# robertknight/ocrs

Hardware: AMD Instinct MI355X
Metric: pages/sec end-to-end (1024x1024) (higher is better)
Workload: dtype f32

## Files before the change

### include/ocrs_amd.h

```cpp
#ifndef OCRS_AMD_H
#define OCRS_AMD_H

#include <stddef.h>
#include <stdint.h>

#if defined(__GNUC__)
#define OCRS_API __attribute__((visibility("default")))
#else
#define OCRS_API
#endif

#ifdef __cplusplus
extern "C" {
#endif

typedef enum ocrs_status {
    OCRS_OK = 0,
    OCRS_ERR_INVALID_ARGUMENT = 1,
    OCRS_ERR_MODEL_NOT_LOADED = 2,
    OCRS_ERR_MODEL_DIMS = 3,
    OCRS_ERR_RUN_FAILED = 4,
    OCRS_ERR_WRONG_OUTPUT = 5,
    OCRS_ERR_IMAGE_SOURCE = 6,
    OCRS_ERR_DEVICE = 7,
    OCRS_ERR_IO = 8,
    OCRS_ERR_CAPACITY = 9
} ocrs_status;

OCRS_API const char* ocrs_last_error(void);

#define OCRS_ABI_VERSION 6u
OCRS_API uint32_t ocrs_abi_version(void);

OCRS_API void ocrs_buffer_free(void* p);

OCRS_API ocrs_status ocrs_device_count(int* n);
OCRS_API ocrs_status ocrs_set_device(int device);
OCRS_API ocrs_status ocrs_get_device(int* device);

OCRS_API ocrs_status ocrs_ctc_beam_search(const float* logp, int t, int c, uint32_t width, int impl, uint32_t** labels,
                                          uint32_t** positions, size_t* n);
OCRS_API ocrs_status ocrs_ctc_beam_search_scored(const float* logp, int t, int c, uint32_t width, int impl, uint32_t** labels,
                                                 uint32_t** positions, size_t* n, double* score, float** step_logp);

OCRS_API ocrs_status ocrs_gru_tile_plan(const int32_t* lengths_desc, size_t n_lines, int hidden, int32_t* n_clusters, int32_t* waves,
                                        int16_t* tiles);

OCRS_API ocrs_status ocrs_coalescer_selftest(int n_threads, int requests_per_thread, int max_active, int max_pages,
                                             long window_us, int fail_every, uint64_t out[5]);

OCRS_API ocrs_status ocrs_set_option(const char* name, long value);
OCRS_API ocrs_status ocrs_option_name(int index, const char** name);

OCRS_API ocrs_status ocrs_device_pool_stats(int device, uint64_t out[12]);
OCRS_API ocrs_status ocrs_device_pool_configure(int device, uint64_t device_cached_cap_bytes, uint64_t pinned_cached_cap_bytes);
OCRS_API ocrs_status ocrs_device_pool_trim(int device);

typedef enum { OCRS_ISOLATION_AUTO = 0, OCRS_ISOLATION_NONE = 1 } ocrs_isolation;
OCRS_API ocrs_status ocrs_device_set_isolation(int device, ocrs_isolation policy);
OCRS_API ocrs_status ocrs_device_isolation(int device, int out[3]);

typedef struct ocrs_model ocrs_model;

OCRS_API ocrs_status ocrs_model_load_file(const char* path, ocrs_model** out);
OCRS_API ocrs_status ocrs_model_load_bytes(const void* data, size_t len, ocrs_model** out);
OCRS_API ocrs_status ocrs_model_load_file_on_device(const char* path, int device, ocrs_model** out);
OCRS_API ocrs_status ocrs_model_load_bytes_on_device(const void* data, size_t len, int device, ocrs_model** out);
OCRS_API ocrs_status ocrs_model_device(const ocrs_model* m, int* device);

// ... 214 lines not shown
```

### ocrs_amd/_lib.py

```python
import ctypes as C
import os

_HERE = os.path.dirname(os.path.abspath(__file__))
LIB_PATH = os.environ.get("OCRS_AMD_LIB") or os.path.join(_HERE, "libocrs_amd.so")

OCRS_OK = 0
STATUS_NAMES = {
    0: "OK", 1: "INVALID_ARGUMENT", 2: "MODEL_NOT_LOADED", 3: "MODEL_DIMS", 4: "RUN_FAILED", 5: "WRONG_OUTPUT",
    6: "IMAGE_SOURCE", 7: "DEVICE", 8: "IO", 9: "CAPACITY",
}

RUN_FN = C.CFUNCTYPE(C.c_int, C.c_void_p, C.POINTER(C.c_float), C.POINTER(C.c_int64), C.POINTER(C.POINTER(C.c_float)),
                     C.POINTER(C.c_int64), C.POINTER(C.c_int))


class EngineParams(C.Structure):
    _fields_ = [("detection_model", C.c_void_p), ("recognition_model", C.c_void_p), ("debug", C.c_int),
                ("decode_method", C.c_int), ("beam_width", C.c_uint32), ("alphabet", C.c_char_p),
                ("allowed_chars", C.c_char_p), ("numerics", C.c_int), ("coalesce", C.c_int), ("coalesce_pages", C.c_int),
                ("coalesce_window_us", C.c_int), ("layout_threads", C.c_int), ("rec_max_pixels", C.c_int64)]


class GroupParams(C.Structure):
    _fields_ = [("detection_model", C.c_void_p), ("detection_model_len", C.c_size_t), ("recognition_model", C.c_void_p),
# ... 12 lines not shown
    _fields_ = [("ch", C.c_uint32), ("top", C.c_int32), ("left", C.c_int32), ("bottom", C.c_int32),
                ("right", C.c_int32)]


class OcrsError(RuntimeError):
    def __init__(self, status, message):
        super().__init__(message)
        self.status = status
        self.status_name = STATUS_NAMES.get(status, str(status))


DECLARED_SYMBOLS = [
    "ocrs_last_error", "ocrs_buffer_free", "ocrs_device_count", "ocrs_set_device", "ocrs_set_option", "ocrs_ctc_beam_search", "ocrs_model_load_file",
    "ocrs_model_load_bytes", "ocrs_model_from_callback", "ocrs_model_input_shape", "ocrs_model_run",
    "ocrs_model_flops", "ocrs_model_free", "ocrs_engine_new", "ocrs_engine_free", "ocrs_image_source_check_bytes",
    "ocrs_engine_prepare_input", "ocrs_engine_prepare_input_device", "ocrs_page_free", "ocrs_page_dims",
    "ocrs_page_image", "ocrs_engine_detect_words", "ocrs_engine_detect_words_batch",
    "ocrs_engine_detect_text_pixels", "ocrs_engine_detection_threshold", "ocrs_engine_find_text_lines",
    "ocrs_engine_find_text_lines_batch",
    "ocrs_engine_recognize_text", "ocrs_engine_recognize_text_batch", "ocrs_engine_recognize_tokens",
    "ocrs_engine_prepare_recognition_input", "ocrs_text_item_rotated_rect", "ocrs_rotated_rect_corners", "ocrs_engine_get_text", "ocrs_device_malloc", "ocrs_device_free",
    "ocrs_device_upload", "ocrs_device_synchronize", "ocrs_device_measure_peaks", "ocrs_engine_enable_timing", "ocrs_stage_count",
    "ocrs_stage_name", "ocrs_engine_stage_times", "ocrs_kernel_class_count", "ocrs_kernel_class_name",
    "ocrs_engine_kernel_stats", "ocrs_engine_set_kernel_timing_mask", "ocrs_gru_tile_plan", "ocrs_host_malloc", "ocrs_host_free", "ocrs_engine_prepare_input_batch",
    "ocrs_get_device", "ocrs_model_load_file_on_device", "ocrs_model_load_bytes_on_device", "ocrs_model_device", "ocrs_engine_device",
    "ocrs_engine_group_new", "ocrs_engine_group_free", "ocrs_engine_group_size", "ocrs_engine_group_member", "ocrs_group_deal",
    "ocrs_group_prepare_input_batch", "ocrs_group_prepare_input_device_batch", "ocrs_group_detect_words_batch",
    "ocrs_group_recognize_text_batch", "ocrs_group_gather", "ocrs_group_final_gather", "ocrs_group_worker_threads", "ocrs_group_last_gather", "ocrs_device_malloc_on", "ocrs_engine_coalesce_stats", "ocrs_coalescer_selftest", "ocrs_engine_kernel_mfma_flops", "ocrs_engine_prepare_input_jpeg", "ocrs_jpeg_decode_rgb", "ocrs_jpeg_info", "ocrs_jpeg_coefficients",
    "ocrs_group_member_stats", "ocrs_numa_parse_cpulist", "ocrs_numa_bind_selftest", "ocrs_engine_recognize_logits", "ocrs_engine_set_option", "ocrs_engine_get_option", "ocrs_option_name", "ocrs_device_pool_stats", "ocrs_device_pool_configure", "ocrs_device_pool_trim",
    "ocrs_device_set_isolation", "ocrs_device_isolation", "ocrs_group_set_replay", "ocrs_abi_version",
    "ocrs_engine_recognize_text_scored", "ocrs_engine_recognize_text_batch_scored", "ocrs_ctc_beam_search_scored",
    "ocrs_engine_run_recognition_ops",
]

ABI_VERSION = 6

_lib = None


def lib():
    global _lib
    if _lib is None:
        if not os.path.exists(LIB_PATH):
            raise OcrsError(7, "libocrs_amd.so is not built: run `python -m ocrs_amd.build` "
                               "(there is no CPU fallback for the HIP engine)")
        L = C.CDLL(LIB_PATH)
        L.ocrs_abi_version.restype = C.c_uint32
# ... 145 lines not shown
```

### ocrs_amd/csrc/abi.cpp

```cpp
#include <cstdio>
#include <fstream>
#include <thread>

#include <atomic>
#include "abi_util.hpp"
#include "coalesce_selftest.hpp"
#include "engine.hpp"
#include "host_pool.hpp"
#include "jpeg.hpp"
#include "kernels.hpp"

using namespace ocrs;
using namespace ocrs::geom;

using namespace ocrs::abi;

extern "C" {

const char* ocrs_last_error(void) { return last_error().c_str(); }

void ocrs_buffer_free(void* p) { free(p); }

ocrs_status ocrs_device_count(int* n) {
    return guarded([&] {
// ... 7 lines not shown
ocrs_status ocrs_set_device(int device) {
    return guarded([&] { select_device(device); });
}

ocrs_status ocrs_get_device(int* device) {
    return guarded([&] {
        if (!device) fail(OCRS_ERR_INVALID_ARGUMENT, "null argument");
        *device = default_device();
    });
}

ocrs_status ocrs_gru_tile_plan(const int32_t* lengths_desc, size_t n_lines, int hidden, int32_t* n_clusters, int32_t* waves,
                               int16_t* tiles) {
    return guarded([&] {
        if (!lengths_desc || !n_clusters || !waves || !tiles || n_lines == 0 || n_lines > (size_t)1 << 20)
            fail(OCRS_ERR_INVALID_ARGUMENT, "bad argument");
        for (size_t i = 0; i < n_lines; i++)
            if (lengths_desc[i] < 1 || (i > 0 && lengths_desc[i] > lengths_desc[i - 1]))
                fail(OCRS_ERR_INVALID_ARGUMENT, "lengths must be positive and descending");
        int ncl = 0;
        if (!k::gru_tile_plan(lengths_desc, (int)n_lines, hidden, &ncl, waves, tiles))
            fail(OCRS_ERR_CAPACITY, "no persistent-kernel plan for this shape (the engine then runs the recurrence as one fused launch per time step)");
        *n_clusters = ncl;
    });
}

ocrs_status ocrs_coalescer_selftest(int n_threads, int requests_per_thread, int max_active, int max_pages, long window_us,
                                    int fail_every, uint64_t out[5]) {
    return guarded([&] {
        if (!out || n_threads < 1 || requests_per_thread < 1 || max_pages < 1) fail(OCRS_ERR_INVALID_ARGUMENT, "bad argument");
        coalescer_selftest(n_threads, requests_per_thread, max_active, max_pages, window_us, fail_every, out);
    });
}

namespace {

void beam_search_hook(const float* logp, int t, int c, uint32_t width, int impl, std::vector<uint32_t>* l,
                      std::vector<uint32_t>* p, double* score, std::vector<float>* step_logp) {
    if (impl == 2 && t > 0) {
        DeviceScope bind(-1);
        if (!k::ctc_beam_supported(c, (int)width)) fail(OCRS_ERR_CAPACITY, "beam search on the GPU supports up to 128 classes and width 128");
        Workspace ws;
        std::vector<int32_t> meta(1 + t + 1);
        meta[0] = t;
        for (int i = 0; i <= t; i++) meta[1 + i] = i;
        int32_t* d_meta = ws.alloc_n<int32_t>(meta.size());
// ... 868 lines not shown
```

### ocrs_amd/csrc/common.cpp

```cpp
#include "common.hpp"

#include <chrono>
#include <climits>
#include <cstdint>
#include <cstdlib>
#include <cstring>

#include <algorithm>
#include <atomic>
#include <condition_variable>
#include <deque>
#include <system_error>

namespace ocrs {

static thread_local std::string g_last_error;

void set_last_error(const std::string& msg) { g_last_error = msg; }
const std::string& last_error() { return g_last_error; }

namespace {
std::atomic<int> g_default_device{0};
thread_local DeviceContext* t_ctx = nullptr;
constexpr int kMaxDevices = 64;
// ... 369 lines not shown
int DeviceContext::cu_count() {
    std::lock_guard<std::mutex> g(lazy_mu_);
    if (!cus_) {
        hipDeviceProp_t prop;
        OCRS_HIP(hipGetDeviceProperties(&prop, device));
        cus_ = prop.multiProcessorCount;
    }
    return cus_;
}

namespace {
struct OptDef { const char* name; const char* env; long def; };
const OptDef kOptDefs[OPT_COUNT] = {
    {"gru_mode", "OCRS_GRU_MODE", GRU_PERSISTENT},
    {"gru_gates", "OCRS_GRU_GATES", 1},
    {"gru_local", "OCRS_GRU_LOCAL", 1},
    {"det_fuse", "OCRS_DET_FUSE", 1},
    {"det_stream", "OCRS_DET_STREAM", 1},
    {"det_rows", "OCRS_DET_ROWS", 1},
    {"ccl_quad", "OCRS_CCL_QUAD", 1},
    {"conv12_fuse", "OCRS_CONV12_FUSE", 1},
    {"conv_flat", "OCRS_CONV_FLAT", 1},
    {"beam_gpu", "OCRS_BEAM_GPU", 1},
    {"numerics", nullptr, 0},
    {"coalesce", nullptr, 2},
    {"coalesce_pages", nullptr, 16},
    {"coalesce_window_us", nullptr, 300},
    {"layout_threads", nullptr, 0},
    {"rec_max_pixels", nullptr, 0},
};
struct OptRange { long lo, hi; long also[4]; };
const OptRange kOptRanges[OPT_COUNT] = {
    {0, 1, {}}, {0, 1, {}}, {0, 1, {}}, {0, 2, {}}, {0, 1, {8, 14, 32}}, {0, 1, {8, 14, 20, 32}}, {0, 1, {}}, {0, 1, {}}, {0, 1, {}}, {0, 1, {}},
    {0, 2, {}}, {0, 64, {}}, {1, 4096, {}}, {0, 10000000, {}}, {0, 4096, {}}, {0, INT64_MAX, {}},
};
bool in_range(int i, long v) {
    const OptRange& r = kOptRanges[i];
    if (v >= r.lo && v <= r.hi) return true;
    for (long a : r.also) if (a && v == a) return true;
    return false;
}
const char* const kRetired[] = {"det_heavy", "det_tail", "gru_waves", "gru_background", "gru_scatter", "gru_gates_pack", "conv_occupancy",
                                "gx_heavy", "gemm_nfast", "conv_a_lds", "gru_heavy", "heavy_priority", "det_mfma"};
std::atomic<long> g_opts[OPT_COUNT];
std::once_flag g_opts_once;
void init_options() {
    for (int i = 0; i < OPT_COUNT; i++) {
        const char* e = kOptDefs[i].env ? getenv(kOptDefs[i].env) : nullptr;
        const long v = e && *e ? strtol(e, nullptr, 10) : kOptDefs[i].def;
        g_opts[i].store(in_range(i, v) ? v : kOptDefs[i].def);
    }
}
int find_option(const char* name, int count = OPT_PUBLIC_COUNT) {
    for (int i = 0; i < count; i++)
        if (name && i != OPT_NUMERICS && strcmp(name, kOptDefs[i].name) == 0) return i;
    return -1;
// ... 173 lines not shown
```

### ocrs_amd/csrc/common.hpp

```cpp
#pragma once
#include <atomic>
#include <hip/hip_runtime.h>

#include <cstdarg>
#include <cstdint>
#include <cstdio>
#include <cstdlib>
#include <chrono>
#include <condition_variable>
#include <cstring>
#include <map>
#include <mutex>
#include <stdexcept>
#include <string>
#include <thread>
#include <vector>

#include "../../include/ocrs_amd.h"

namespace ocrs {

struct Error : std::runtime_error {
    ocrs_status status;
    Error(ocrs_status s, const std::string& msg) : std::runtime_error(msg), status(s) {}
// ... 94 lines not shown

DeviceContext& device_context(int device);
int default_device();
void select_device(int device);
DeviceContext& ctx();

class DeviceScope {
  public:
    explicit DeviceScope(int device);
    ~DeviceScope();
    DeviceScope(const DeviceScope&) = delete;
    DeviceScope& operator=(const DeviceScope&) = delete;

  private:
    DeviceContext* prev_;
    int restore_ = -1;
};

inline DevicePool& pool() { return ctx().pool; }
inline HostPool& host_pool() { return ctx().host_pool; }
inline hipStream_t heavy_stream() { return ctx().heavy_stream(); }

enum Option { OPT_GRU_MODE = 0, OPT_GRU_GATES, OPT_GRU_LOCAL, OPT_DET_FUSE, OPT_DET_STREAM, OPT_DET_ROWS, OPT_CCL_QUAD,
              OPT_CONV12_FUSE, OPT_CONV_FLAT, OPT_BEAM_GPU, OPT_PUBLIC_COUNT,
              OPT_NUMERICS = OPT_PUBLIC_COUNT,
              OPT_COALESCE, OPT_COALESCE_PAGES, OPT_COALESCE_WINDOW_US,
              OPT_LAYOUT_THREADS, OPT_REC_MAX_PIXELS,
              OPT_COUNT };
struct Tuning { long v[OPT_COUNT]; };
Tuning default_tuning();
int set_option(const char* name, long value);
int set_option(Tuning& t, const char* name, long value);
bool get_option(const Tuning& t, const char* name, long* value);
const char* option_name(int i);
class TuningScope {
  public:
    explicit TuningScope(const Tuning* t);
    ~TuningScope();
    TuningScope(const TuningScope&) = delete;
    TuningScope& operator=(const TuningScope&) = delete;
  private:
    const Tuning* prev_;
};
const Tuning* current_tuning();
enum { GRU_PERSISTENT = 0, GRU_STEP = 1 };
int option(Option o);

// ... 192 lines not shown
```

### ocrs_amd/csrc/kernels.hpp

```cpp
#pragma once
#include <vector>
#include <hip/hip_runtime.h>

#include <cstdint>

namespace ocrs {
namespace jpeg { struct Coefficients; }
namespace k {

void prepare_image(const void* d_pixels, bool is_u8, bool chans_last, int h, int w, int chans, float* d_out,
                   hipStream_t s);
void resize_pages_to_model(const float* const* d_src_ptrs, int n, int sh, int sw, int vh, int vw, float* d_dst,
                           int dh, int dw, hipStream_t s);
bool resize_threshold(const float* d_prob, int n, int mh, int mw, int sh, int sw, float thr, uint8_t* d_mask,
                      float* d_map, int h, int w, hipStream_t s, int32_t* d_labels = nullptr, int32_t* d_zero_a = nullptr,
                      int32_t* d_zero_b = nullptr);
void threshold_only(const float* d_prob, float thr, uint8_t* d_mask, int64_t count, hipStream_t s);

struct CclBuffers {
    int32_t* labels;
    int32_t* row_counts;
    int32_t* row_offsets;
    int32_t* n_roots;
    int32_t* roots;
// ... 67 lines not shown
void padcat(const float* skip, int n, int sh, int sw, int cs, const float* x, int h, int w, int cx, float* y,
            hipStream_t s);
void sigmoid(const float* x, float* y, int64_t count, hipStream_t s);
void conv1x1_cout1(const float* x, int64_t pixels, int cin, const float* wt, const float* bias, int relu, int do_sigmoid,
                   float* y, hipStream_t s);
void to_seq(const float* x, int n, int w, int c, float* y, hipStream_t s);
void gru_gates(const float* gx, const float* gh, float* h, float* y, int T, int N, int H, int step, hipStream_t s);
bool log_softmax_argmax(const float* logits, int64_t rows, int c, const uint8_t* d_excluded ,
                        float* logp, int32_t* labels, hipStream_t s, float* maxlp = nullptr);
void to_seq_packed(const float* x, int n, int T, int c, const int32_t* d_pos, const int32_t* d_off, float* y,
                   hipStream_t s);
void gru_gates_packed(const float* gx, const float* gh, float* h, float* y, const int32_t* d_Tm, const int32_t* d_off,
                      int64_t R, int Mcap, int active, int H, int step, hipStream_t s);
bool gru_step_fused(const float* gx, const float* wh, const float* bh, const float* hT_in, float* hT_out, float* y,
                    const int32_t* d_Tm, const int32_t* d_off, int64_t R, int Mcap, int active, int H, int step,
                    hipStream_t s);
size_t gru_persistent_sync_words(int M);
size_t gru_persistent_exchange_bytes(const int32_t* h_Tm, int M, int H);
bool gru_persistent_supported(const int32_t* h_Tm, int M, int Tmax, int64_t R, int H);
bool gru_tile_plan(const int32_t* h_Tm, int M, int H, int* ncl, int* waves, int16_t* tiles );
hipError_t gru_persistent_prepare(float* hx, const int32_t* h_Tm, int M, int H, hipStream_t s);
bool gru_persistent(const float* gx, const float* wh, const float* bh, float* y, float* hx, const int32_t* d_Tm, const int32_t* d_off,
                    const int32_t* h_Tm, int64_t R, int M, int Tmax, int H, uint32_t* d_sync, hipStream_t s);
bool gru_general_tile_plan(const int32_t* h_Tm, int M, int Tmax, int H, int cap, int* ncl, int16_t* tiles , int kernel );
size_t gru_split_exchange_bytes(const int32_t* h_Tm, int M, int H, int np);
bool gru_split_supported(const int32_t* h_Tm, int M, int Tmax, int64_t R, int H, int np);
hipError_t gru_split_prepare(uint16_t* hx, const int32_t* h_Tm, int M, int H, int np, hipStream_t s);
bool gru_persistent_split(const float* gx, const float* wh, const float* bh, float* y, uint16_t* hx, const int32_t* d_Tm, const int32_t* d_off,
                          const int32_t* h_Tm, int64_t R, int M, int Tmax, int H, int np, uint32_t* d_sync, hipStream_t s);
void ctc_collapse_packed(const int32_t* labels, const int32_t* d_Tm, const int32_t* d_off, int M, int Tmax,
                         uint32_t* out_labels, uint32_t* out_pos, int32_t* out_count, hipStream_t s);
void ctc_collapse_scored_packed(const int32_t* labels, const float* maxlp, const int32_t* d_Tm, const int32_t* d_off, int M,
                                int Tmax, uint32_t* out_labels, uint32_t* out_pos, float* out_logp, int32_t* out_count,
                                double* out_score, hipStream_t s);
void argmax_rows(const float* x, int64_t rows, int c, const uint8_t* d_excluded, int32_t* labels, hipStream_t s);
bool ctc_beam_supported(int C, int width);
size_t ctc_beam_arena_entries(int Tmax, int width);
bool ctc_beam_packed(const float* logp, const int32_t* d_Tm, const int32_t* d_off, int M, int Tmax, int C, int width,
                     const uint8_t* d_excluded, int2* d_nodes, int2* d_posn, uint32_t* out_labels, uint32_t* out_pos,
                     int32_t* out_count, hipStream_t s, double* out_score = nullptr, float* out_logp = nullptr);
void ctc_collapse(const int32_t* labels, int T, int N, uint32_t* out_labels, uint32_t* out_pos, int32_t* out_count,
                  hipStream_t s);

struct RaggedView {
    int G;
    int H;
// ... 57 lines not shown
```

### ocrs_amd/csrc/kernels_gru.hip

```cpp
#include <algorithm>
#include <cstdlib>
#include <map>
#include <mutex>
#include <vector>

#include "common.hpp"
#include "kernels.hpp"
#include "spec_math.hpp"

namespace ocrs {
namespace k {

typedef float f32x4 __attribute__((ext_vector_type(4)));
typedef unsigned u32x2 __attribute__((ext_vector_type(2)));

namespace {

constexpr int kMaxSlots = 128;

struct GruParams {
    const float* gx;
    const float* wh;
    const float* bh;
    float* y;
// ... 311 lines not shown
        if (!early) issue_state<H>(hxb, ub, kq, nxt);
        if (!await_state<H>(p, hxb, ub, kq, nxt)) return -1;
#ifdef OCRS_GRU_PROBE
        pr_wait += __builtin_readcyclecounter() - pt3;
#endif
        s = ns;
        i = ni;
        return 1;
    };
    for (;;) {
        if (item(bufA, bufB) <= 0) break;
        if (item(bufB, bufA) <= 0) break;
    }
#ifdef OCRS_GRU_PROBE
    if (cid == 0 && ub == 0 && lane == 0)
        printf("probe fp32 wave %d local %d tiles %d: items %llu, cycles per item %llu = transposes + issue %llu | chain %llu | gates + stores %llu | wait %llu\n", wave, (int)local,
               (t0 >= 0) + (t1 >= 0) + (t2 >= 0) + (t3 >= 0), (unsigned long long)pr_items, (unsigned long long)((__builtin_readcyclecounter() - pr_t0) / pr_items),
               (unsigned long long)(pr_tr / pr_items), (unsigned long long)(pr_mma / pr_items), (unsigned long long)(pr_gate / pr_items), (unsigned long long)(pr_wait / pr_items));
#endif
}



template <int H>
__device__ __forceinline__ f32x4 gate_chain(int lane, const float (&w)[H / 4], const float* lds_w, int g, const f32x4& bias) {
    f32x4 acc = bias;
    const f32x4* ap = reinterpret_cast<const f32x4*>(lds_w) + g * (H / 16) * 64 + lane;
    f32x4 a = ap[0];
#pragma unroll
    for (int blk = 0; blk < H / 16; blk++) {
        f32x4 na = a;
        if (blk + 1 < H / 16) na = ap[(blk + 1) * 64];
#pragma unroll
        for (int e = 0; e < 4; e++) acc = __builtin_amdgcn_mfma_f32_16x16x4f32(a[e], w[4 * blk + e], acc, 0, 0, 0);
        a = na;
    }
    return acc;
}

template <int H, bool FAST>
__global__ void __launch_bounds__(256)
gru_gates_kernel(GruParams p) {
    extern __shared__ __attribute__((aligned(16))) float lds_w[];
    asm volatile("v_accvgpr_write_b32 a200, 0" ::: "a200");
    constexpr int UB = H / 16;
    const int b = blockIdx.x;
// ... 108 lines not shown
                const float rg = sigmoid_g<FAST>(gr[r] + a.r[r]);
                const float zg = sigmoid_g<FAST>(gz[r] + a.z[r]);
                const float ng = tanh_g<FAST>(fmaf(rg, a.n[r], gn[r]));
                const float hv = fmaf(zg, hp[r] - ng, ng);
                hn[r] = __float_as_uint(hv) == kUnwritten ? __uint_as_float(0x7FC00000u) : hv;
            }
            const uint32_t o = active ? ((blk0 + s) * (H / 16) + ub) * 1024u + i16 * 64u + kq * 16u : 0xFFFFFFF0u;
            float t[4];
            transpose4(hn, t);
            const f32x4 ht = {t[0], t[1], t[2], t[3]};
            if (local) store_local(hxb, o, ht);
            else store_through(hxb, o, ht);
            store_local(yb, active ? out_off : 0xFFFFFFF0u, hn);
            if (active) hp = hn;
            gr = ngr; gz = ngz; gn = ngn; out_off = nout_off; active = nactive;
        }
    }
}


}

constexpr int kMaxGrid = 4096;
static size_t gru_gates_lds_bytes(int H, int Tmax) {
    return (size_t)H * 48 * sizeof(float) + (size_t)(((Tmax + 1) + 3) & ~3) * sizeof(int) + 3 * 64 * 16 + 16;
}
static size_t gru_general_lds_bytes(int H, int Tmax) { return (size_t)H * 48 * sizeof(float) + ((size_t)Tmax + 1) * sizeof(int); }
size_t gru_persistent_sync_words(int) { return kMaxGrid + 1; }

static int64_t gru_tile_blocks(const int32_t* h_Tm, int M) {
    int64_t tb = 0;
    for (int m = 0; m < M; m += 16) tb += h_Tm[m];
    return tb;
}
size_t gru_persistent_exchange_bytes(const int32_t* h_Tm, int M, int H) { return (size_t)2 * (size_t)gru_tile_blocks(h_Tm, M) * 16 * H * sizeof(float); }

hipError_t gru_persistent_prepare(float* hx, const int32_t* h_Tm, int M, int H, hipStream_t s) {
    return M > 0 ? hipMemsetAsync(hx, 0xFF, gru_persistent_exchange_bytes(h_Tm, M, H), s) : hipSuccess;
}

static int gru_resident_capacity(int H, bool gates, size_t lds) {
    static std::mutex mu;
    static std::map<int, int> cache;
    int dev = 0;
    if (hipGetDevice(&dev) != hipSuccess) return 0;
    const int key = dev * 8 + (gates ? 4 : 0) + (H == 256 ? 2 : H == 128 ? 1 : 0);
    {
        std::lock_guard<std::mutex> g(mu);
        auto it = cache.find(key);
        if (it != cache.end()) return it->second;
    }
    hipDeviceProp_t prop;
    if (hipGetDeviceProperties(&prop, dev) != hipSuccess) return 0;
    int per_cu = 0;
    hipError_t e;
    if (gates) {
        e = H == 256 ? hipOccupancyMaxActiveBlocksPerMultiprocessor(&per_cu, gru_gates_kernel<256, false>, 256, lds)
          : H == 128 ? hipOccupancyMaxActiveBlocksPerMultiprocessor(&per_cu, gru_gates_kernel<128, false>, 256, lds)
                     : hipOccupancyMaxActiveBlocksPerMultiprocessor(&per_cu, gru_gates_kernel<64, false>, 256, lds);
    } else {
        e = H == 256 ? hipOccupancyMaxActiveBlocksPerMultiprocessor(&per_cu, gru_persistent_kernel<256, false>, 256, lds)
          : H == 128 ? hipOccupancyMaxActiveBlocksPerMultiprocessor(&per_cu, gru_persistent_kernel<128, false>, 256, lds)
                     : hipOccupancyMaxActiveBlocksPerMultiprocessor(&per_cu, gru_persistent_kernel<64, false>, 256, lds);
    }
    if (e != hipSuccess) { (void)hipGetLastError(); per_cu = 0; }
    const int cap = prop.multiProcessorCount * (per_cu > 0 ? 1 : 0);
    std::lock_guard<std::mutex> g(mu);
    cache[key] = cap;
    return cap;
}

static bool gru_plan(int M, int Tmax, int H, int* ncl, int max_blocks = 256) {
    if (H != 256 && H != 128 && H != 64) return false;
    const int ntiles = (M + 15) / 16;
    const int UB = H / 16;
    max_blocks = max_blocks > 256 ? 256 : max_blocks;
    max_blocks -= max_blocks % (8 * UB);
    if (max_blocks < 8 * UB) return false;
    int max_ncl = max_blocks / UB / 2;
    if (ntiles > 16 * max_ncl) max_ncl *= 2;
    if (ntiles > 16 * max_ncl || 4 * max_ncl > kMaxSlots) return false;
    *ncl = (ntiles + 3) / 4 < max_ncl ? (ntiles + 3) / 4 : max_ncl;
    return gru_general_lds_bytes(H, Tmax) <= 64 * 1024;
}

static const int kRoundCost[3][5] = {{0, 63, 101, 150, 200}, {0, 54, 91, 128, 170}, {0, 44, 68, 99, 135}};
static void gru_assign_tiles(const int32_t* h_Tm, int M, int ncl, int16_t* tiles, int kernel = 0) {
    const int ntiles = (M + 15) / 16, nslots = 4 * ncl;
    const int* round = kRoundCost[kernel >= 0 && kernel < 3 ? kernel : 0];
    for (int i = 0; i < nslots * 4; i++) tiles[i] = -1;
    std::vector<int> cnt(nslots, 0);
    auto cost = [&](int slot, int extra_len) {
        int64_t tot = 0;
        int len[5], n = cnt[slot];
        for (int i = 0; i < n; i++) len[i] = h_Tm[tiles[slot * 4 + i] * 16];
        if (extra_len > 0) len[n++] = extra_len;
        for (int i = n - 1, below = 0; i >= 0; i--) {
            tot += (int64_t)(len[i] - below) * round[i + 1];
            below = len[i];
        }
        return tot;
    };
    for (int k = 0; k < ntiles; k++) {
        const int len = h_Tm[k * 16];
        int best = -1;
        int64_t best_cost = 0;
        for (int sl = 0; sl < nslots; sl++) {
            if (cnt[sl] >= 4) continue;
            const int64_t cs = cost(sl, len);
            if (best < 0 || cs < best_cost) { best = sl; best_cost = cs; }
        }
        tiles[best * 4 + cnt[best]++] = (int16_t)k;
    }
}

bool gru_tile_plan(const int32_t* h_Tm, int M, int H, int* ncl, int* waves, int16_t* tiles ) {
    for (int i = 0; i < kMaxSlots * 4; i++) tiles[i] = -1;
    *waves = 4;
    if (M <= 0 || !gru_plan(M, h_Tm[0], H, ncl, 256)) return false;
    gru_assign_tiles(h_Tm, M, *ncl, tiles);
    return true;
}

bool gru_general_tile_plan(const int32_t* h_Tm, int M, int Tmax, int H, int cap, int* ncl, int16_t* tiles, int kernel) {
    if (M <= 0 || !gru_plan(M, Tmax, H, ncl, cap)) return false;
    if (tiles) gru_assign_tiles(h_Tm, M, *ncl, tiles, kernel);
    return true;
}

bool gru_persistent_supported(const int32_t* h_Tm, int M, int Tmax, int64_t R, int H) {
    int ncl;
    if (H != 256 && H != 128 && H != 64) return false;
    return M > 0 && (uint64_t)R * 2 * H * sizeof(float) < (uint64_t(1) << 32) && (uint64_t)gru_persistent_exchange_bytes(h_Tm, M, H) < (uint64_t(1) << 32) &&
           gru_plan(M, Tmax, H, &ncl, gru_resident_capacity(H, false, gru_general_lds_bytes(H, Tmax)));
}

static bool gru_gates_plan(int M, int Tmax, int H, int* ncl) {
    if (H != 256 && H != 128 && H != 64) return false;
    if (gru_gates_lds_bytes(H, Tmax) > 64 * 1024) return false;
    const int ntiles = (M + 15) / 16, UB = H / 16;
    int cap = gru_resident_capacity(H, true, gru_gates_lds_bytes(H, Tmax));
    cap = cap > 256 ? 256 : cap;
    cap -= cap % (8 * UB);
    if (cap < 8 * UB || ntiles > cap / UB / 2) return false;
    *ncl = ntiles;
    return true;
}

template <int H>
static void launch_gates(bool fast, dim3 grid, size_t lds, hipStream_t s, const GruParams& g) {
    if (fast) hipLaunchKernelGGL((gru_gates_kernel<H, true>), grid, dim3(256), lds, s, g);
    else hipLaunchKernelGGL((gru_gates_kernel<H, false>), grid, dim3(256), lds, s, g);
}
template <int H>
static void launch_general(bool fast, dim3 grid, size_t lds, hipStream_t s, const GruParams& g) {
    if (fast) hipLaunchKernelGGL((gru_persistent_kernel<H, true>), grid, dim3(256), lds, s, g);
    else hipLaunchKernelGGL((gru_persistent_kernel<H, false>), grid, dim3(256), lds, s, g);
}

bool gru_persistent(const float* gx, const float* wh, const float* bh, float* y, float* hx, const int32_t* d_Tm, const int32_t* d_off,
                    const int32_t* h_Tm, int64_t R, int M, int Tmax, int H, uint32_t* d_sync, hipStream_t s) {
    if (M <= 0) return true;
    if (!hx || !gru_persistent_supported(h_Tm, M, Tmax, R, H)) return false;
    const bool fast = option(OPT_NUMERICS) != 0;
    GruParams p{};
    p.gx = gx; p.wh = wh; p.bh = bh; p.y = y; p.hx = hx; p.Tm = d_Tm; p.off = d_off;
    std::vector<int32_t> base((M + 15) / 16 + 1, 0);
    for (size_t k = 0; k + 1 < base.size(); k++) base[k + 1] = base[k] + h_Tm[k * 16];
    p.TB = base.back();
    p.place = d_sync;
    p.sync = d_sync + kMaxGrid;
    p.R = R; p.M = M; p.Tmax = Tmax;
    p.prio = 3;
    p.spin_limit = 1u << 21;
    p.allow_local = option(OPT_GRU_LOCAL) != 0;
    const int UB = H / 16;
    if (option(OPT_GRU_GATES) && gru_gates_plan(M, Tmax, H, &p.ncl)) {
        for (int k = 0; k < p.ncl; k++) p.tbase[k] = base[k];
        const dim3 grid(8 * UB * ((2 * p.ncl + 7) / 8));
        const size_t lds = gru_gates_lds_bytes(H, Tmax);
        OCRS_HIP(hipMemsetAsync(d_sync, 0, gru_persistent_sync_words(M) * sizeof(uint32_t), s));
        if (H == 256) launch_gates<256>(fast, grid, lds, s, p);
        else if (H == 128) launch_gates<128>(fast, grid, lds, s, p);
        else launch_gates<64>(fast, grid, lds, s, p);
        return true;
    }
    if (!gru_plan(M, Tmax, H, &p.ncl, gru_resident_capacity(H, false, gru_general_lds_bytes(H, Tmax)))) return false;
    gru_assign_tiles(h_Tm, M, p.ncl, p.tiles);
    for (int i = 0; i < 16 * p.ncl; i++) p.tbase[i] = p.tiles[i] >= 0 ? base[p.tiles[i]] : 0;
    const dim3 grid(8 * UB * ((2 * p.ncl + 7) / 8));
    if (grid.x > (unsigned)kMaxGrid) return false;
    const size_t lds = gru_general_lds_bytes(H, Tmax);
    OCRS_HIP(hipMemsetAsync(d_sync, 0, gru_persistent_sync_words(M) * sizeof(uint32_t), s));
    if (H == 256) launch_general<256>(fast, grid, lds, s, p);
    else if (H == 128) launch_general<128>(fast, grid, lds, s, p);
    else launch_general<64>(fast, grid, lds, s, p);
    return true;
}

}
}
```

Measured before the change: 271.3.

## Add weights-in-registers persistent GRU kernel for hidden size 256

Adds a new persistent GRU recurrence kernel for H=256 that keeps each wave's slice of the recurrent weight matrix in registers. It stages the previous hidden state through double-buffered LDS rows and overlaps loading the next item's state with the current MFMA chain. It is selected by a new default-on option when the gates kernel is not used, and gets its own tile-dealing plan with new round costs. It removes the per-step weight reads from LDS/global, at the cost of very high register pressure and lower occupancy. It also adds a launch counter and a plan query to the public ABI.

Measured after the change: 275.1, median of 6. 1.01x the previous value.

```diff
diff --git a/include/ocrs_amd.h b/include/ocrs_amd.h
--- a/include/ocrs_amd.h
+++ b/include/ocrs_amd.h
@@ -45,6 +45,11 @@
 
 OCRS_API ocrs_status ocrs_gru_tile_plan(const int32_t* lengths_desc, size_t n_lines, int hidden, int32_t* n_clusters, int32_t* waves,
                                         int16_t* tiles);
+
+OCRS_API ocrs_status ocrs_gru_wreg_tile_plan(const int32_t* lengths_desc, size_t n_lines, int hidden, int32_t* n_clusters,
+                                             int16_t* tiles, int32_t* round_cost);
+
+OCRS_API ocrs_status ocrs_gru_launch_counts(uint64_t out[3]);
 
 OCRS_API ocrs_status ocrs_coalescer_selftest(int n_threads, int requests_per_thread, int max_active, int max_pages,
                                              long window_us, int fail_every, uint64_t out[5]);
diff --git a/ocrs_amd/_lib.py b/ocrs_amd/_lib.py
--- a/ocrs_amd/_lib.py
+++ b/ocrs_amd/_lib.py
@@ -58,7 +58,7 @@
     "ocrs_engine_prepare_recognition_input", "ocrs_text_item_rotated_rect", "ocrs_rotated_rect_corners", "ocrs_engine_get_text", "ocrs_device_malloc", "ocrs_device_free",
     "ocrs_device_upload", "ocrs_device_synchronize", "ocrs_device_measure_peaks", "ocrs_engine_enable_timing", "ocrs_stage_count",
     "ocrs_stage_name", "ocrs_engine_stage_times", "ocrs_kernel_class_count", "ocrs_kernel_class_name",
-    "ocrs_engine_kernel_stats", "ocrs_engine_set_kernel_timing_mask", "ocrs_gru_tile_plan", "ocrs_host_malloc", "ocrs_host_free", "ocrs_engine_prepare_input_batch",
+    "ocrs_engine_kernel_stats", "ocrs_engine_set_kernel_timing_mask", "ocrs_gru_tile_plan", "ocrs_gru_wreg_tile_plan", "ocrs_gru_launch_counts", "ocrs_host_malloc", "ocrs_host_free", "ocrs_engine_prepare_input_batch",
     "ocrs_get_device", "ocrs_model_load_file_on_device", "ocrs_model_load_bytes_on_device", "ocrs_model_device", "ocrs_engine_device",
     "ocrs_engine_group_new", "ocrs_engine_group_free", "ocrs_engine_group_size", "ocrs_engine_group_member", "ocrs_group_deal",
     "ocrs_group_prepare_input_batch", "ocrs_group_prepare_input_device_batch", "ocrs_group_detect_words_batch",
diff --git a/ocrs_amd/csrc/abi.cpp b/ocrs_amd/csrc/abi.cpp
--- a/ocrs_amd/csrc/abi.cpp
+++ b/ocrs_amd/csrc/abi.cpp
@@ -53,6 +53,28 @@
         if (!k::gru_tile_plan(lengths_desc, (int)n_lines, hidden, &ncl, waves, tiles))
             fail(OCRS_ERR_CAPACITY, "no persistent-kernel plan for this shape (the engine then runs the recurrence as one fused launch per time step)");
         *n_clusters = ncl;
+    });
+}
+
+ocrs_status ocrs_gru_wreg_tile_plan(const int32_t* lengths_desc, size_t n_lines, int hidden, int32_t* n_clusters, int16_t* tiles,
+                                    int32_t* round_cost) {
+    return guarded([&] {
+        if (!lengths_desc || !n_clusters || !tiles || !round_cost || n_lines == 0 || n_lines > (size_t)1 << 20)
+            fail(OCRS_ERR_INVALID_ARGUMENT, "bad argument");
+        for (size_t i = 0; i < n_lines; i++)
+            if (lengths_desc[i] < 1 || (i > 0 && lengths_desc[i] > lengths_desc[i - 1]))
+                fail(OCRS_ERR_INVALID_ARGUMENT, "lengths must be positive and descending");
+        int ncl = 0;
+        if (!k::gru_wreg_tile_plan(lengths_desc, (int)n_lines, hidden, &ncl, tiles, round_cost))
+            fail(OCRS_ERR_CAPACITY, "no weights-in-registers plan for this shape (the engine then runs the general persistent kernel)");
+        *n_clusters = ncl;
+    });
+}
+
+ocrs_status ocrs_gru_launch_counts(uint64_t out[3]) {
+    return guarded([&] {
+        if (!out) fail(OCRS_ERR_INVALID_ARGUMENT, "null argument");
+        k::gru_launch_counts(out);
     });
 }
 
diff --git a/ocrs_amd/csrc/common.cpp b/ocrs_amd/csrc/common.cpp
--- a/ocrs_amd/csrc/common.cpp
+++ b/ocrs_amd/csrc/common.cpp
@@ -415,6 +415,7 @@
     {"conv12_fuse", "OCRS_CONV12_FUSE", 1},
     {"conv_flat", "OCRS_CONV_FLAT", 1},
     {"beam_gpu", "OCRS_BEAM_GPU", 1},
+    {"gru_wreg", "OCRS_GRU_WREG", 1},
     {"numerics", nullptr, 0},
     {"coalesce", nullptr, 2},
     {"coalesce_pages", nullptr, 16},
@@ -424,7 +425,7 @@
 };
 struct OptRange { long lo, hi; long also[4]; };
 const OptRange kOptRanges[OPT_COUNT] = {
-    {0, 1, {}}, {0, 1, {}}, {0, 1, {}}, {0, 2, {}}, {0, 1, {8, 14, 32}}, {0, 1, {8, 14, 20, 32}}, {0, 1, {}}, {0, 1, {}}, {0, 1, {}}, {0, 1, {}},
+    {0, 1, {}}, {0, 1, {}}, {0, 1, {}}, {0, 2, {}}, {0, 1, {8, 14, 32}}, {0, 1, {8, 14, 20, 32}}, {0, 1, {}}, {0, 1, {}}, {0, 1, {}}, {0, 1, {}}, {0, 1, {}},
     {0, 2, {}}, {0, 64, {}}, {1, 4096, {}}, {0, 10000000, {}}, {0, 4096, {}}, {0, INT64_MAX, {}},
 };
 bool in_range(int i, long v) {
diff --git a/ocrs_amd/csrc/common.hpp b/ocrs_amd/csrc/common.hpp
--- a/ocrs_amd/csrc/common.hpp
+++ b/ocrs_amd/csrc/common.hpp
@@ -140,7 +140,7 @@
 inline hipStream_t heavy_stream() { return ctx().heavy_stream(); }
 
 enum Option { OPT_GRU_MODE = 0, OPT_GRU_GATES, OPT_GRU_LOCAL, OPT_DET_FUSE, OPT_DET_STREAM, OPT_DET_ROWS, OPT_CCL_QUAD,
-              OPT_CONV12_FUSE, OPT_CONV_FLAT, OPT_BEAM_GPU, OPT_PUBLIC_COUNT,
+              OPT_CONV12_FUSE, OPT_CONV_FLAT, OPT_BEAM_GPU, OPT_GRU_WREG, OPT_PUBLIC_COUNT,
               OPT_NUMERICS = OPT_PUBLIC_COUNT,
               OPT_COALESCE, OPT_COALESCE_PAGES, OPT_COALESCE_WINDOW_US,
               OPT_LAYOUT_THREADS, OPT_REC_MAX_PIXELS,
diff --git a/ocrs_amd/csrc/kernels.hpp b/ocrs_amd/csrc/kernels.hpp
--- a/ocrs_amd/csrc/kernels.hpp
+++ b/ocrs_amd/csrc/kernels.hpp
@@ -113,6 +113,8 @@
 hipError_t gru_persistent_prepare(float* hx, const int32_t* h_Tm, int M, int H, hipStream_t s);
 bool gru_persistent(const float* gx, const float* wh, const float* bh, float* y, float* hx, const int32_t* d_Tm, const int32_t* d_off,
                     const int32_t* h_Tm, int64_t R, int M, int Tmax, int H, uint32_t* d_sync, hipStream_t s);
+void gru_launch_counts(uint64_t out[3]);
+bool gru_wreg_tile_plan(const int32_t* h_Tm, int M, int H, int* ncl, int16_t* tiles , int32_t* round_cost );
 bool gru_general_tile_plan(const int32_t* h_Tm, int M, int Tmax, int H, int cap, int* ncl, int16_t* tiles , int kernel );
 size_t gru_split_exchange_bytes(const int32_t* h_Tm, int M, int H, int np);
 bool gru_split_supported(const int32_t* h_Tm, int M, int Tmax, int64_t R, int H, int np);
diff --git a/ocrs_amd/csrc/kernels_gru.hip b/ocrs_amd/csrc/kernels_gru.hip
--- a/ocrs_amd/csrc/kernels_gru.hip
+++ b/ocrs_amd/csrc/kernels_gru.hip
@@ -1,4 +1,5 @@
 #include <algorithm>
+#include <atomic>
 #include <cstdlib>
 #include <map>
 #include <mutex>
@@ -357,6 +358,241 @@
 
 
 
+struct WregItem {
+    f32x4 pc[4];
+    f32x4 gr, gz, gn;
+    uint32_t out_off;
+    uint32_t hx_off;
+    uint32_t prev_off;
+    bool has_prev;
+    bool active;
+};
+
+template <int H>
+__device__ __forceinline__ void wreg_issue_meta(const GruParams& p, int dir, int ub, int wave, int tile, int tbase, int tm, const int* off_l,
+                                                int s, int i16, int kq, WregItem& L) {
+    const int m = tile * 16 + i16;
+    L.active = tm > s;
+    const int t = dir ? tm - 1 - s : s;
+    const int64_t row = L.active ? (int64_t)off_l[t] + m : 0;
+    L.out_off = (uint32_t)((row * 2 * H + dir * H + ub * 16 + kq * 4) * sizeof(float));
+    L.has_prev = L.active && s > 0;
+    const uint32_t blk = (uint32_t)(dir * p.TB + tbase + s);
+    L.hx_off = (blk * (H / 16) + ub) * 1024u + i16 * 64u + kq * 16u;
+    const float* g = p.gx + ((int64_t)dir * p.R + row) * 3 * H + ub * 16 + kq * 4;
+    L.gr = *reinterpret_cast<const f32x4*>(g);
+    L.gz = *reinterpret_cast<const f32x4*>(g + H);
+    L.gn = *reinterpret_cast<const f32x4*>(g + 2 * H);
+    L.prev_off = L.has_prev ? ((blk - 1u) * (H / 16) + 4u * wave) * 1024u + i16 * 64u + kq * 16u : 0xFFFFF000u;
+}
+
+__device__ __forceinline__ void wreg_issue_state(__amdgpu_buffer_rsrc_t hx, WregItem& L) {
+#pragma unroll
+    for (int j = 0; j < 4; j++) L.pc[j] = load_bypass(hx, L.prev_off + j * 1024u);
+}
+
+__device__ __forceinline__ bool wreg_state_ready(const WregItem& L) {
+    unsigned mx = 0;
+#pragma unroll
+    for (int j = 0; j < 4; j++)
+#pragma unroll
+        for (int e = 0; e < 4; e++) mx = max(mx, __float_as_uint(L.pc[j][e]));
+    return !__any(mx == kUnwritten);
+}
+
+__device__ __forceinline__ void wreg_settle(WregItem& L) {
+#pragma unroll
+    for (int j = 0; j < 4; j++) asm volatile("" : "+v"(L.pc[j]));
+}
+
+__device__ __forceinline__ bool wreg_await_state(const GruParams& p, __amdgpu_buffer_rsrc_t hx, WregItem& L) {
+    if (__builtin_expect(wreg_state_ready(L), 1)) {
+        wreg_settle(L);
+        return true;
+    }
+    uint32_t spins = 0;
+    do {
+        __builtin_amdgcn_s_sleep(2);
+        if (spins >= 4u) {
+            const uint32_t n = spins < 36u ? (spins >> 2) : 9u;
+            for (uint32_t z = 0; z < n; z++) __builtin_amdgcn_s_sleep(16);
+        }
+        if ((spins & 255u) == 255u) {
+            gu32* err = (gu32*)p.sync;
+            const uint32_t e = __builtin_amdgcn_readfirstlane(__hip_atomic_load(err, __ATOMIC_RELAXED, __HIP_MEMORY_SCOPE_AGENT));
+            if (e != 0 || spins >= p.spin_limit) {
+                __hip_atomic_store(err, 3u, __ATOMIC_RELAXED, __HIP_MEMORY_SCOPE_AGENT);
+                return false;
+            }
+        }
+        wreg_issue_state(hx, L);
+        spins++;
+    } while (!wreg_state_ready(L));
+    wreg_settle(L);
+    return true;
+}
+
+template <int H, bool FAST>
+__global__ void __launch_bounds__(256)
+gru_persistent_kernel_wreg(GruParams p) {
+    extern __shared__ __attribute__((aligned(16))) float lds_s[];
+    constexpr int WG = H / 64;
+    constexpr int RS = H + 16;
+    const int b = blockIdx.x;
+    const int q = b >> 3;
+    const int wg = q % WG;
+    const int cid = (q / WG) * 8 + (b & 7);
+    if (cid >= 2 * p.ncl) return;
+    const int dir = cid & 1, cl = cid >> 1;
+    const int tid = threadIdx.x;
+    const int lane = tid & 63;
+    const int wave = __builtin_amdgcn_readfirstlane(tid >> 6);
+    const int i16 = lane & 15, kq = lane >> 4;
+    const int ub = wg * 4 + wave;
+    uint32_t xcc;
+    asm volatile("s_getreg_b32 %0, hwreg(HW_REG_XCC_ID, 0, 4)" : "=s"(xcc));
+    if (tid == 0) __hip_atomic_store((gu32*)p.place + cid * WG + wg, xcc + 1u, __ATOMIC_RELAXED, __HIP_MEMORY_SCOPE_AGENT);
+    const float* __restrict__ whd = p.wh + (int64_t)dir * H * 3 * H;
+    const float* __restrict__ bhd = p.bh + (int64_t)dir * 3 * H;
+    const int j0 = ub * 16;
+    int* off_l = reinterpret_cast<int*>(lds_s + 2 * 16 * RS);
+    int* abort_w = off_l + p.Tmax + 1;
+    for (int i = tid; i <= p.Tmax; i += 256) off_l[i] = p.off[i];
+    if (tid == 0) *abort_w = 0;
+    float w[3][H / 4];
+    {
+        const float* wl = whd + (int64_t)kq * 3 * H + j0 + i16;
+#pragma unroll
+        for (int g = 0; g < 3; g++)
+#pragma unroll
+            for (int s4 = 0; s4 < H / 4; s4++) w[g][s4] = wl[(int64_t)s4 * 12 * H + g * H];
+    }
+    const f32x4 br = *reinterpret_cast<const f32x4*>(bhd + j0 + kq * 4);
+    const f32x4 bz = *reinterpret_cast<const f32x4*>(bhd + H + j0 + kq * 4);
+    const f32x4 bn = *reinterpret_cast<const f32x4*>(bhd + 2 * H + j0 + kq * 4);
+    const int t0 = p.tiles[cl * 4 + 0], t1 = p.tiles[cl * 4 + 1], t2 = p.tiles[cl * 4 + 2], t3 = p.tiles[cl * 4 + 3];
+    auto tile_of = [&](int i) { return i == 0 ? t0 : i == 1 ? t1 : i == 2 ? t2 : t3; };
+    int tmr[4], tT[4];
+#pragma unroll
+    for (int i = 0; i < 4; i++) {
+        const int m = tile_of(i) * 16 + i16;
+        tmr[i] = (tile_of(i) >= 0 && m < p.M) ? p.Tm[m] : 0;
+        tT[i] = __builtin_amdgcn_readfirstlane(tmr[i]);
+    }
+    auto sel = [](const int (&a)[4], int i) { return i == 0 ? a[0] : i == 1 ? a[1] : i == 2 ? a[2] : i == 3 ? a[3] : 0; };
+    __syncthreads();
+    if (p.prio >= 3) __builtin_amdgcn_s_setprio(3);
+    else if (p.prio == 2) __builtin_amdgcn_s_setprio(2);
+    else if (p.prio == 1) __builtin_amdgcn_s_setprio(1);
+    if (tT[0] <= 0) return;
+    bool local;
+    {
+        const gu32* pl = (const gu32*)p.place + cid * WG;
+        uint32_t v = xcc + 1u;
+        for (uint32_t spins = 0;; spins++) {
+            if (lane < WG) v = __hip_atomic_load(pl + lane, __ATOMIC_RELAXED, __HIP_MEMORY_SCOPE_AGENT);
+            if (!__any(v == 0u)) break;
+            __builtin_amdgcn_s_sleep(8);
+            if (spins >= p.spin_limit) {
+                __hip_atomic_store((gu32*)p.sync, 4u, __ATOMIC_RELAXED, __HIP_MEMORY_SCOPE_AGENT);
+                *abort_w = 1;
+                break;
+            }
+        }
+        local = !__any(v != xcc + 1u) && p.allow_local;
+    }
+    const __amdgpu_buffer_rsrc_t yb = __builtin_amdgcn_make_buffer_rsrc(p.y, 0, (int)(uint32_t)(p.R * 2 * H * sizeof(float)), 0x00020000);
+    const __amdgpu_buffer_rsrc_t hxb = __builtin_amdgcn_make_buffer_rsrc(p.hx, 0, (int)((uint32_t)p.TB * 2u * (H / 16) * 1024u), 0x00020000);
+    const int tb0 = p.tbase[cl * 4 + 0], tb1 = p.tbase[cl * 4 + 1], tb2 = p.tbase[cl * 4 + 2], tb3 = p.tbase[cl * 4 + 3];
+    auto tbase_of = [&](int i) { return i == 0 ? tb0 : i == 1 ? tb1 : i == 2 ? tb2 : tb3; };
+    const int hsw = (0x1230 >> (4 * (i16 >> 2))) & 3;
+    float* const row0 = lds_s + i16 * RS;
+    int s = 0, i = 0;
+#ifdef OCRS_GRU_PROBE
+    uint64_t pr_stage = 0, pr_issue = 0, pr_mma = 0, pr_gate = 0, pr_wait = 0, pr_items = 0, pr_t0 = __builtin_readcyclecounter();
+#endif
+    WregItem bufA, bufB;
+    wreg_issue_meta<H>(p, dir, ub, wave, tile_of(0), tbase_of(0), tmr[0], off_l, 0, i16, kq, bufA);
+    {
+        const f32x4 zero = {0.0f, 0.0f, 0.0f, 0.0f};
+#pragma unroll
+        for (int j = 0; j < 4; j++) bufA.pc[j] = zero;
+    }
+    auto item = [&](WregItem& cur, WregItem& nxt, const int par) -> int {
+        int ns = s, ni = i + 1;
+        if (sel(tT, ni) <= s) { ns = s + 1; ni = 0; }
+        const bool have_next = sel(tT, ni) > ns;
+        const bool early = have_next && ni != i;
+        float* const rowp = row0 + par * 16 * RS;
+#ifdef OCRS_GRU_PROBE
+        const uint64_t pt0 = __builtin_readcyclecounter();
+#endif
+#pragma unroll
+        for (int j = 0; j < 4; j++)
+#pragma unroll
+            for (int r = 0; r < 4; r++) rowp[(4 * wave + j) * 16 + ((r ^ hsw) << 2) + kq] = cur.pc[j][r];
+        __syncthreads();
+        if (*abort_w) return -1;
+#ifdef OCRS_GRU_PROBE
+        const uint64_t pt1 = __builtin_readcyclecounter();
+#endif
+        if (have_next) wreg_issue_meta<H>(p, dir, ub, wave, tile_of(ni), tbase_of(ni), sel(tmr, ni), off_l, ns, i16, kq, nxt);
+        if (early) wreg_issue_state(hxb, nxt);
+        const f32x4* bp = reinterpret_cast<const f32x4*>(rowp + ((kq ^ hsw) << 2));
+        f32x4 acc_r = br, acc_z = bz, acc_n = bn;
+#ifdef OCRS_GRU_PROBE
+        const uint64_t pt2 = __builtin_readcyclecounter();
+#endif
+        f32x4 bv = bp[0];
+#pragma unroll
+        for (int blk = 0; blk < H / 16; blk++) {
+            f32x4 nb = bv;
+            if (blk + 1 < H / 16) nb = bp[(blk + 1) * 4];
+#pragma unroll
+            for (int e = 0; e < 4; e++) {
+                acc_r = __builtin_amdgcn_mfma_f32_16x16x4f32(w[0][4 * blk + e], bv[e], acc_r, 0, 0, 0);
+                acc_z = __builtin_amdgcn_mfma_f32_16x16x4f32(w[1][4 * blk + e], bv[e], acc_z, 0, 0, 0);
+                acc_n = __builtin_amdgcn_mfma_f32_16x16x4f32(w[2][4 * blk + e], bv[e], acc_n, 0, 0, 0);
+            }
+            bv = nb;
+        }
+#ifdef OCRS_GRU_PROBE
+        asm volatile("" :: "v"(acc_r), "v"(acc_z), "v"(acc_n));
+        const uint64_t pt3 = __builtin_readcyclecounter();
+#endif
+        f32x4 hp;
+#pragma unroll
+        for (int r = 0; r < 4; r++) hp[r] = rowp[ub * 16 + ((r ^ hsw) << 2) + kq];
+        __builtin_amdgcn_s_waitcnt(0x0F70);
+        const f32x4 hn = epilogue_store<H, FAST>(hxb, GateAcc{acc_r, acc_z, acc_n}, cur.gr, cur.gz, cur.gn, hp, cur.hx_off, cur.active, local);
+        store_local(yb, cur.active ? cur.out_off : 0xFFFFFFF0u, hn);
+#ifdef OCRS_GRU_PROBE
+        const uint64_t pt4 = __builtin_readcyclecounter();
+        pr_stage += pt1 - pt0; pr_issue += pt2 - pt1; pr_mma += pt3 - pt2; pr_gate += pt4 - pt3; pr_items++;
+#endif
+        if (!have_next) return 0;
+        if (!early) wreg_issue_state(hxb, nxt);
+        if (!wreg_await_state(p, hxb, nxt)) *abort_w = 1;
+#ifdef OCRS_GRU_PROBE
+        pr_wait += __builtin_readcyclecounter() - pt4;
+#endif
+        s = ns;
+        i = ni;
+        return 1;
+    };
+    for (;;) {
+        if (item(bufA, bufB, 0) <= 0) break;
+        if (item(bufB, bufA, 1) <= 0) break;
+    }
+#ifdef OCRS_GRU_PROBE
+    if (cid == 0 && wg == 0 && lane == 0)
+        printf("probe wreg wave %d local %d tiles %d: items %llu, cycles per item %llu = stage + barrier %llu | meta + issue %llu | chain %llu | gates + stores %llu | wait %llu\n", wave,
+               (int)local, (t0 >= 0) + (t1 >= 0) + (t2 >= 0) + (t3 >= 0), (unsigned long long)pr_items, (unsigned long long)((__builtin_readcyclecounter() - pr_t0) / pr_items),
+               (unsigned long long)(pr_stage / pr_items), (unsigned long long)(pr_issue / pr_items), (unsigned long long)(pr_mma / pr_items), (unsigned long long)(pr_gate / pr_items),
+               (unsigned long long)(pr_wait / pr_items));
+#endif
+}
+
 template <int H>
 __device__ __forceinline__ f32x4 gate_chain(int lane, const float (&w)[H / 4], const float* lds_w, int g, const f32x4& bias) {
     f32x4 acc = bias;
@@ -511,10 +747,18 @@
 }
 
 constexpr int kMaxGrid = 4096;
+enum { kGruGeneral = 0, kGruGates = 1, kGruWreg = 2 };
+static std::atomic<uint64_t> g_gru_launches[3];
+void gru_launch_counts(uint64_t out[3]) {
+    for (int i = 0; i < 3; i++) out[i] = g_gru_launches[i].load(std::memory_order_relaxed);
+}
 static size_t gru_gates_lds_bytes(int H, int Tmax) {
     return (size_t)H * 48 * sizeof(float) + (size_t)(((Tmax + 1) + 3) & ~3) * sizeof(int) + 3 * 64 * 16 + 16;
 }
 static size_t gru_general_lds_bytes(int H, int Tmax) { return (size_t)H * 48 * sizeof(float) + ((size_t)Tmax + 1) * sizeof(int); }
+static size_t gru_wreg_lds_bytes(int H, int Tmax) {
+    return (size_t)2 * 16 * (H + 16) * sizeof(float) + ((size_t)Tmax + 2) * sizeof(int);
+}
 size_t gru_persistent_sync_words(int) { return kMaxGrid + 1; }
 
 static int64_t gru_tile_blocks(const int32_t* h_Tm, int M) {
@@ -528,12 +772,12 @@
     return M > 0 ? hipMemsetAsync(hx, 0xFF, gru_persistent_exchange_bytes(h_Tm, M, H), s) : hipSuccess;
 }
 
-static int gru_resident_capacity(int H, bool gates, size_t lds) {
+static int gru_resident_capacity(int H, int kind, size_t lds) {
     static std::mutex mu;
     static std::map<int, int> cache;
     int dev = 0;
     if (hipGetDevice(&dev) != hipSuccess) return 0;
-    const int key = dev * 8 + (gates ? 4 : 0) + (H == 256 ? 2 : H == 128 ? 1 : 0);
+    const int key = dev * 16 + kind * 4 + (H == 256 ? 2 : H == 128 ? 1 : 0);
     {
         std::lock_guard<std::mutex> g(mu);
         auto it = cache.find(key);
@@ -543,7 +787,9 @@
     if (hipGetDeviceProperties(&prop, dev) != hipSuccess) return 0;
     int per_cu = 0;
     hipError_t e;
-    if (gates) {
+    if (kind == kGruWreg) {
+        e = H == 256 ? hipOccupancyMaxActiveBlocksPerMultiprocessor(&per_cu, gru_persistent_kernel_wreg<256, false>, 256, lds) : hipErrorInvalidValue;
+    } else if (kind == kGruGates) {
         e = H == 256 ? hipOccupancyMaxActiveBlocksPerMultiprocessor(&per_cu, gru_gates_kernel<256, false>, 256, lds)
           : H == 128 ? hipOccupancyMaxActiveBlocksPerMultiprocessor(&per_cu, gru_gates_kernel<128, false>, 256, lds)
                      : hipOccupancyMaxActiveBlocksPerMultiprocessor(&per_cu, gru_gates_kernel<64, false>, 256, lds);
@@ -573,10 +819,9 @@
     return gru_general_lds_bytes(H, Tmax) <= 64 * 1024;
 }
 
-static const int kRoundCost[3][5] = {{0, 63, 101, 150, 200}, {0, 54, 91, 128, 170}, {0, 44, 68, 99, 135}};
-static void gru_assign_tiles(const int32_t* h_Tm, int M, int ncl, int16_t* tiles, int kernel = 0) {
-    const int ntiles = (M + 15) / 16, nslots = 4 * ncl;
-    const int* round = kRoundCost[kernel >= 0 && kernel < 3 ? kernel : 0];
+static const int kRoundCost[4][5] = {{0, 63, 101, 150, 200}, {0, 54, 91, 128, 170}, {0, 44, 68, 99, 135}, {0, 53, 93, 140, 187}};
+static void gru_deal_tiles(const int32_t* h_Tm, int M, int nslots, const int* round, int16_t* tiles) {
+    const int ntiles = (M + 15) / 16;
     for (int i = 0; i < nslots * 4; i++) tiles[i] = -1;
     std::vector<int> cnt(nslots, 0);
     auto cost = [&](int slot, int extra_len) {
@@ -602,6 +847,34 @@
         tiles[best * 4 + cnt[best]++] = (int16_t)k;
     }
 }
+static void gru_assign_tiles(const int32_t* h_Tm, int M, int ncl, int16_t* tiles, int kernel = 0) {
+    gru_deal_tiles(h_Tm, M, 4 * ncl, kRoundCost[kernel >= 0 && kernel < 3 ? kernel : 0], tiles);
+}
+
+constexpr int kWregRound = 3;
+static bool gru_wreg_plan(int M, int Tmax, int H, int* ncl, int max_blocks = 256) {
+    if (H != 256) return false;
+    const int ntiles = (M + 15) / 16;
+    const int WG = H / 64;
+    max_blocks = max_blocks > 256 ? 256 : max_blocks;
+    max_blocks -= max_blocks % (8 * WG);
+    if (max_blocks < 8 * WG) return false;
+    int max_ncl = max_blocks / WG / 2;
+    if (ntiles > 4 * max_ncl) max_ncl *= 2;
+    if (ntiles > 4 * max_ncl || max_ncl > kMaxSlots) return false;
+    *ncl = ntiles < max_ncl ? ntiles : max_ncl;
+    return gru_wreg_lds_bytes(H, Tmax) <= 64 * 1024;
+}
+static void gru_wreg_assign_tiles(const int32_t* h_Tm, int M, int ncl, int16_t* tiles) {
+    gru_deal_tiles(h_Tm, M, ncl, kRoundCost[kWregRound], tiles);
+}
+bool gru_wreg_tile_plan(const int32_t* h_Tm, int M, int H, int* ncl, int16_t* tiles , int32_t* round_cost ) {
+    for (int i = 0; i < kMaxSlots * 4; i++) tiles[i] = -1;
+    for (int i = 0; i < 5; i++) round_cost[i] = kRoundCost[kWregRound][i];
+    if (M <= 0 || !gru_wreg_plan(M, h_Tm[0], H, ncl, 256)) return false;
+    gru_wreg_assign_tiles(h_Tm, M, *ncl, tiles);
+    return true;
+}
 
 bool gru_tile_plan(const int32_t* h_Tm, int M, int H, int* ncl, int* waves, int16_t* tiles ) {
     for (int i = 0; i < kMaxSlots * 4; i++) tiles[i] = -1;
@@ -621,14 +894,14 @@
     int ncl;
     if (H != 256 && H != 128 && H != 64) return false;
     return M > 0 && (uint64_t)R * 2 * H * sizeof(float) < (uint64_t(1) << 32) && (uint64_t)gru_persistent_exchange_bytes(h_Tm, M, H) < (uint64_t(1) << 32) &&
-           gru_plan(M, Tmax, H, &ncl, gru_resident_capacity(H, false, gru_general_lds_bytes(H, Tmax)));
+           gru_plan(M, Tmax, H, &ncl, gru_resident_capacity(H, kGruGeneral, gru_general_lds_bytes(H, Tmax)));
 }
 
 static bool gru_gates_plan(int M, int Tmax, int H, int* ncl) {
     if (H != 256 && H != 128 && H != 64) return false;
     if (gru_gates_lds_bytes(H, Tmax) > 64 * 1024) return false;
     const int ntiles = (M + 15) / 16, UB = H / 16;
-    int cap = gru_resident_capacity(H, true, gru_gates_lds_bytes(H, Tmax));
+    int cap = gru_resident_capacity(H, kGruGates, gru_gates_lds_bytes(H, Tmax));
     cap = cap > 256 ? 256 : cap;
     cap -= cap % (8 * UB);
     if (cap < 8 * UB || ntiles > cap / UB / 2) return false;
@@ -640,6 +913,11 @@
 static void launch_gates(bool fast, dim3 grid, size_t lds, hipStream_t s, const GruParams& g) {
     if (fast) hipLaunchKernelGGL((gru_gates_kernel<H, true>), grid, dim3(256), lds, s, g);
     else hipLaunchKernelGGL((gru_gates_kernel<H, false>), grid, dim3(256), lds, s, g);
+}
+template <int H>
+static void launch_wreg(bool fast, dim3 grid, size_t lds, hipStream_t s, const GruParams& g) {
+    if (fast) hipLaunchKernelGGL((gru_persistent_kernel_wreg<H, true>), grid, dim3(256), lds, s, g);
+    else hipLaunchKernelGGL((gru_persistent_kernel_wreg<H, false>), grid, dim3(256), lds, s, g);
 }
 template <int H>
 static void launch_general(bool fast, dim3 grid, size_t lds, hipStream_t s, const GruParams& g) {
@@ -672,9 +950,23 @@
         if (H == 256) launch_gates<256>(fast, grid, lds, s, p);
         else if (H == 128) launch_gates<128>(fast, grid, lds, s, p);
         else launch_gates<64>(fast, grid, lds, s, p);
+        g_gru_launches[kGruGates]++;
         return true;
     }
-    if (!gru_plan(M, Tmax, H, &p.ncl, gru_resident_capacity(H, false, gru_general_lds_bytes(H, Tmax)))) return false;
+    if (option(OPT_GRU_WREG) && gru_wreg_plan(M, Tmax, H, &p.ncl, gru_resident_capacity(H, kGruWreg, gru_wreg_lds_bytes(H, Tmax)))) {
+        const int WG = H / 64;
+        const dim3 grid(8 * WG * ((2 * p.ncl + 7) / 8));
+        if (grid.x <= (unsigned)kMaxGrid) {
+            gru_wreg_assign_tiles(h_Tm, M, p.ncl, p.tiles);
+            for (int i = 0; i < 4 * p.ncl; i++) p.tbase[i] = p.tiles[i] >= 0 ? base[p.tiles[i]] : 0;
+            const size_t lds = gru_wreg_lds_bytes(H, Tmax);
+            OCRS_HIP(hipMemsetAsync(d_sync, 0, gru_persistent_sync_words(M) * sizeof(uint32_t), s));
+            launch_wreg<256>(fast, grid, lds, s, p);
+            g_gru_launches[kGruWreg]++;
+            return true;
+        }
+    }
+    if (!gru_plan(M, Tmax, H, &p.ncl, gru_resident_capacity(H, kGruGeneral, gru_general_lds_bytes(H, Tmax)))) return false;
     gru_assign_tiles(h_Tm, M, p.ncl, p.tiles);
     for (int i = 0; i < 16 * p.ncl; i++) p.tbase[i] = p.tiles[i] >= 0 ? base[p.tiles[i]] : 0;
     const dim3 grid(8 * UB * ((2 * p.ncl + 7) / 8));
@@ -684,6 +976,7 @@
     if (H == 256) launch_general<256>(fast, grid, lds, s, p);
     else if (H == 128) launch_general<128>(fast, grid, lds, s, p);
     else launch_general<64>(fast, grid, lds, s, p);
+    g_gru_launches[kGruGeneral]++;
     return true;
 }
 
```
